# aiven/tiered-storage-for-apache-kafka

Hardware: AMD Instinct MI355X
Metric: GiB/s segment chunk transform (Zstd+AES+CRC), 4MiB chunks (higher is better)
Workload: dtype u8

## Files before the change

### tiered-storage-for-apache-kafka_amd/csrc/zstd_enc_dev.h

```cpp
#define LANES 64
#define UNI(x) ((uint32_t)__builtin_amdgcn_readfirstlane((uint32_t)(x)))
#ifdef HIPEMU
#define ZS_GLOBAL
#else
#define ZS_GLOBAL __attribute__((address_space(1)))
#endif
typedef const ZS_GLOBAL uint8_t* gbytes_t;
typedef ZS_GLOBAL uint32_t* gwords_t;
struct __attribute__((packed)) zs_u64u { uint64_t v; };
struct __attribute__((packed)) zs_u32u { uint32_t v; };
__device__ static inline uint64_t gld64(gbytes_t p) { return reinterpret_cast<const ZS_GLOBAL zs_u64u*>(p)->v; }
__device__ static inline uint32_t gld32(gbytes_t p) { return reinterpret_cast<const ZS_GLOBAL zs_u32u*>(p)->v; }
__device__ static inline uint4 ld128a(const uint8_t* p) { return *reinterpret_cast<const uint4*>(p); }
#ifdef HIPEMU
__device__ static inline void zs_put_seq(zs_seq* p, uint32_t offBase, uint32_t litLength, uint32_t mlBase, uint32_t litPos) { zs_seq q; q.offBase = offBase; q.litLength = litLength; q.mlBase = mlBase; q.litPos = litPos; *p = q; }
#else
typedef uint32_t zs_u32x4 __attribute__((ext_vector_type(4)));
__device__ static inline uint4 ld128a(gbytes_t p) { const zs_u32x4 t = *reinterpret_cast<const ZS_GLOBAL zs_u32x4*>(p); return make_uint4(t.x, t.y, t.z, t.w); }
__device__ static inline void zs_put_seq(ZS_GLOBAL zs_seq* p, uint32_t offBase, uint32_t litLength, uint32_t mlBase, uint32_t litPos) {
    zs_u32x4 t; t.x = offBase; t.y = litLength; t.z = mlBase; t.w = litPos;
    *reinterpret_cast<ZS_GLOBAL zs_u32x4*>(p) = t;
}
#endif
template <class T> __device__ static inline T* uni_ptr(T* p) {
// ... 4 lines not shown
#define ZS_RING 4096u
#define ZS_RWM (ZS_RING / 4 - 1)
#define ZS_FILL 2048u
#define ZS_SAFE 384u
#ifndef ZS_WAVES_PER_SIMD
#define ZS_WAVES_PER_SIMD 6
#endif
#define ZS_SCR 1024u
#define ZS_NOINLINE __attribute__((noinline))

#ifdef TSX_PROF
__shared__ unsigned long long g_prof[24];
__shared__ unsigned long long g_prof_take;
static unsigned long long* g_prof_out = nullptr;
extern "C" void tsx_debug_set_prof(void* dev_ptr) { g_prof_out = (unsigned long long*)dev_ptr; }
#define ZS_PROF_PARAM , unsigned long long* __restrict__ prof_out
#define ZS_PROF_ARG , prof_out
#define ZS_PROF_LAUNCH_ARG , g_prof_out
#else
#define ZS_PROF_PARAM
#define ZS_PROF_ARG
#define ZS_PROF_LAUNCH_ARG
#endif
#if defined(TSX_PROF) && !defined(TSX_PROF2)
#define PT(k) do { const unsigned long long now_ = (unsigned long long)clock64(); if (threadIdx.x == 0) { g_prof[k] += now_ - g_prof[23]; g_prof[23] = now_; } } while (0)
#define PCNT(k, v) do { if (threadIdx.x == 0) g_prof[k] += (v); } while (0)
#define PTW(k) do { asm volatile("s_waitcnt vmcnt(0) lgkmcnt(0)" ::: "memory"); PT(k); } while (0)
#else
#define PT(k) do {} while (0)
#define PCNT(k, v) do {} while (0)
#define PTW(k) do {} while (0)
#endif

__device__ static const uint8_t kLLbits[36] = {0,0,0,0,0,0,0,0,0,0,0,0,0,0,0,0,1,1,1,1,2,2,3,3,4,6,7,8,9,10,11,12,13,14,15,16};
__device__ static const uint8_t kMLbits[53] = {0,0,0,0,0,0,0,0,0,0,0,0,0,0,0,0,0,0,0,0,0,0,0,0,0,0,0,0,0,0,0,0,1,1,1,1,2,2,3,3,4,4,5,7,8,9,10,11,12,13,14,15,16};
__device__ static const short kLLdefaultNorm[36] = {4,3,2,2,2,2,2,2,2,2,2,2,2,1,1,1,2,2,2,2,2,2,2,2,2,3,2,1,1,1,1,1,-1,-1,-1,-1};
__device__ static const short kOFdefaultNorm[29] = {1,1,1,1,1,1,2,2,2,1,1,1,1,1,1,1,1,1,1,1,1,1,1,1,-1,-1,-1,-1,-1};
__device__ static const short kMLdefaultNorm[53] = {1,4,3,2,2,2,2,2,2,1,1,1,1,1,1,1,1,1,1,1,1,1,1,1,1,1,1,1,1,1,1,1,1,1,1,1,1,1,1,1,1,1,1,1,1,1,-1,-1,-1,-1,-1,-1,-1};
__device__ static const uint8_t kLLcode[64] = {0,1,2,3,4,5,6,7,8,9,10,11,12,13,14,15,16,16,17,17,18,18,19,19,20,20,20,20,21,21,21,21,
    22,22,22,22,22,22,22,22,23,23,23,23,23,23,23,23,24,24,24,24,24,24,24,24,24,24,24,24,24,24,24,24};
__device__ static const uint8_t kMLcode[128] = {0,1,2,3,4,5,6,7,8,9,10,11,12,13,14,15,16,17,18,19,20,21,22,23,24,25,26,27,28,29,30,31,
    32,32,33,33,34,34,35,35,36,36,36,36,37,37,37,37,38,38,38,38,38,38,38,38,39,39,39,39,39,39,39,39,
    40,40,40,40,40,40,40,40,40,40,40,40,40,40,40,40,41,41,41,41,41,41,41,41,41,41,41,41,41,41,41,41,
    42,42,42,42,42,42,42,42,42,42,42,42,42,42,42,42,42,42,42,42,42,42,42,42,42,42,42,42,42,42,42,42};
__device__ static const uint32_t kRtb[8] = {0, 473195, 504333, 520860, 550000, 700000, 750000, 830000};

__device__ static inline uint32_t hb32(uint32_t v) { return 31u - (uint32_t)__clz((int)v); }
__device__ static inline uint64_t ld64(const uint8_t* p) { uint64_t v; __builtin_memcpy(&v, p, 8); return v; }
__device__ static inline uint32_t LLcode(uint32_t ll) { return ll > 63 ? hb32(ll) + 19 : kLLcode[ll]; }
__device__ static inline uint32_t MLcode(uint32_t ml) { return ml > 127 ? hb32(ml) + 36 : kMLcode[ml]; }

struct HufTable { uint16_t val[256]; uint8_t nb[256]; uint32_t tableLog, maxSym; };
struct FseTable { uint16_t state[512]; uint32_t dnb[56]; int32_t dfs[56]; uint32_t tableLog; };

enum {
    ZS_SCAL_HUF_HSIZE = 0,
    ZS_SCAL_HUF_USEOLD = 1,
    ZS_SCAL_HUF_FAIL = 2,
    ZS_SCAL_SEQ_QOFF = 3,
    ZS_SCAL_SEQ_COUNTSIZE = 4,
    ZS_SCAL_HUF_BC = 4,
    ZS_SCAL_NEWHUF = 8,
    ZS_SCAL_MULT = 15
};
struct EncLds {
    int hufRepeat[2];
    uint32_t scal[16];
    union alignas(16) {
        struct {
            union { FseTable ll; HufTable huf[2]; };
            FseTable of;
            union {
                FseTable ml;
                uint32_t hist[256];
            };
            uint32_t hist2[256];
            uint8_t tableSymbol[512];
            uint16_t cumul[64];
            short norm[64];
        };
        struct {
            uint32_t ring[ZS_RING / 4 + 4];
            uint8_t scr[2 * ZS_SCR];
        } p;
        struct {
            tsx_gf128 tab[256];
            uint32_t t0[256];
        } g;
        uint32_t crcTab[4 * 256];
    };
};

#ifdef HIPEMU
// ... 24 lines not shown
```

### tiered-storage-for-apache-kafka_amd/csrc/zstd_enc_entropy.h

```cpp
struct BitW { uint8_t* start; uint8_t* p; uint8_t* end; uint64_t acc; uint32_t n; bool overflow; };
__device__ static inline void bw_init(BitW& b, uint8_t* dst, uint8_t* end) { b.start = b.p = dst; b.end = end; b.acc = 0; b.n = 0; b.overflow = false; }
__device__ static inline void bw_add(BitW& b, uint64_t v, uint32_t nb) {
    if (!nb) return;
    b.acc |= (v & ((1ull << nb) - 1)) << b.n;
    b.n += nb;
    while (b.n >= 8) { if (b.p < b.end) *b.p++ = (uint8_t)b.acc; else b.overflow = true; b.acc >>= 8; b.n -= 8; }
}
__device__ static inline uint32_t bw_close(BitW& b) {
    bw_add(b, 1, 1);
    if (b.n) { if (b.p < b.end) *b.p++ = (uint8_t)b.acc; else b.overflow = true; b.n = 0; }
    return (uint32_t)(b.p - b.start);
}

__device__ static uint32_t fse_minTableLog(uint32_t srcSize, uint32_t maxSym) {
    uint32_t a = hb32(srcSize) + 1, b = hb32(maxSym) + 2;
    return a < b ? a : b;
}
__device__ static uint32_t fse_optimalTableLog(uint32_t maxTableLog, uint32_t srcSize, uint32_t maxSym, uint32_t minus) {
    uint32_t maxBitsSrc = hb32(srcSize - 1) - minus, tableLog = maxTableLog, minBits = fse_minTableLog(srcSize, maxSym);
    if (maxBitsSrc < tableLog) tableLog = maxBitsSrc;
    if (minBits > tableLog) tableLog = minBits;
    if (tableLog < 5) tableLog = 5;
    if (tableLog > 12) tableLog = 12;
    return tableLog;
// ... 73 lines not shown
    uint32_t bitStream = 0; int bitCount = 0; uint32_t symbol = 0; const uint32_t alphabetSize = maxSym + 1; int previousIs0 = 0;
    bitStream += (tableLog - 5) << bitCount; bitCount += 4;
    remaining = tableSize + 1; threshold = tableSize; nbBits = (int)tableLog + 1;
    while (symbol < alphabetSize && remaining > 1) {
        if (previousIs0) {
            uint32_t start = symbol;
            while (symbol < alphabetSize && !norm[symbol]) symbol++;
            if (symbol == alphabetSize) break;
            while (symbol >= start + 24) { start += 24; bitStream += 0xFFFFU << bitCount; out[0] = (uint8_t)bitStream; out[1] = (uint8_t)(bitStream >> 8); out += 2; bitStream >>= 16; }
            while (symbol >= start + 3) { start += 3; bitStream += 3U << bitCount; bitCount += 2; }
            bitStream += (symbol - start) << bitCount; bitCount += 2;
            if (bitCount > 16) { out[0] = (uint8_t)bitStream; out[1] = (uint8_t)(bitStream >> 8); out += 2; bitStream >>= 16; bitCount -= 16; }
        }
        {   int c = norm[symbol++];
            const int mx = (2 * threshold - 1) - remaining;
            remaining -= c < 0 ? -c : c;
            c++;
            if (c >= threshold) c += mx;
            bitStream += (uint32_t)c << bitCount;
            bitCount += nbBits;
            bitCount -= (c < mx);
            previousIs0 = (c == 1);
            if (remaining < 1) return 0;
            while (remaining < threshold) { nbBits--; threshold >>= 1; }
        }
        if (bitCount > 16) { out[0] = (uint8_t)bitStream; out[1] = (uint8_t)(bitStream >> 8); out += 2; bitStream >>= 16; bitCount -= 16; }
    }
    if (remaining != 1) return 0;
    out[0] = (uint8_t)bitStream; out[1] = (uint8_t)(bitStream >> 8);
    out += (bitCount + 7) / 8;
    return (uint32_t)(out - out0);
}

__device__ ZS_NOINLINE static void fse_buildCTable(FseTable& ct, const short* norm, uint32_t maxSym, uint32_t tableLog, uint16_t* cumul, uint8_t* tableSymbol) {
    const uint32_t tableSize = 1u << tableLog, tableMask = tableSize - 1, step = (tableSize >> 1) + (tableSize >> 3) + 3;
    uint32_t highThreshold = tableSize - 1, u;
    ct.tableLog = tableLog;
    cumul[0] = 0;
    for (u = 1; u <= maxSym + 1; u++) {
        if (norm[u - 1] == -1) { cumul[u] = (uint16_t)(cumul[u - 1] + 1); tableSymbol[highThreshold--] = (uint8_t)(u - 1); }
        else cumul[u] = (uint16_t)(cumul[u - 1] + (uint32_t)norm[u - 1]);
    }
    cumul[maxSym + 1] = (uint16_t)(tableSize + 1);
    {   uint32_t position = 0;
        for (uint32_t symbol = 0; symbol <= maxSym; symbol++) {
            const int freq = norm[symbol];
            for (int n = 0; n < freq; n++) {
                tableSymbol[position] = (uint8_t)symbol;
                position = (position + step) & tableMask;
                while (position > highThreshold) position = (position + step) & tableMask;
            }
        }
    }
    for (u = 0; u < tableSize; u++) { const uint8_t s = tableSymbol[u]; ct.state[cumul[s]++] = (uint16_t)(tableSize + u); }
    {   uint32_t total = 0;
        for (uint32_t s = 0; s <= maxSym; s++) {
            const int nv = norm[s];
            if (nv == 0) { ct.dnb[s] = ((tableLog + 1) << 16) - (1u << tableLog); ct.dfs[s] = 0; }
            else if (nv == -1 || nv == 1) { ct.dnb[s] = (tableLog << 16) - (1u << tableLog); ct.dfs[s] = (int)(total - 1); total++; }
            else {
                const uint32_t maxBitsOut = tableLog - hb32((uint32_t)nv - 1), minStatePlus = (uint32_t)nv << maxBitsOut;
                ct.dnb[s] = (maxBitsOut << 16) - minStatePlus; ct.dfs[s] = (int)(total - (uint32_t)nv); total += (uint32_t)nv;
            }
        }
    }
}
__device__ static inline uint32_t fse_init2(const FseTable& ct, uint32_t symbol) {
    const uint32_t dnb = ct.dnb[symbol];
    const uint32_t nbBitsOut = (dnb + (1u << 15)) >> 16;
    const uint32_t value = (nbBitsOut << 16) - dnb;
    return ct.state[(value >> nbBitsOut) + ct.dfs[symbol]];
}
__device__ static inline void fse_encode(BitW& b, const FseTable& ct, uint32_t& value, uint32_t symbol) {
    const uint32_t nbBitsOut = (value + ct.dnb[symbol]) >> 16;
    bw_add(b, value, nbBitsOut);
    value = ct.state[(value >> nbBitsOut) + ct.dfs[symbol]];
}

__device__ ZS_NOINLINE static uint32_t huf_writeCTable(uint8_t* dst, const HufTable& ct, uint32_t maxSym, uint32_t huffLog, EncLds& L) {
    uint8_t* const hw = reinterpret_cast<uint8_t*>(L.hist2);
    for (uint32_t n = 0; n < maxSym; n++) { const uint32_t nb = ct.nb[n]; hw[n] = nb ? (uint8_t)(huffLog + 1 - nb) : 0; }
    uint32_t hSize = 0;
    {
        uint8_t* op = dst + 1; const uint32_t wtSize = maxSym;
        uint32_t maxSV = ZS_HUF_TABLELOG_MAX; uint32_t* cnt = L.hist2 + 68;
        if (wtSize > 1) {
// ... 13 lines not shown
                else {
                    BitW b; bw_init(b, op, op + 512);
                    const uint8_t* ip = hw + wtSize; uint32_t s1, s2;
                    if (wtSize & 1) { s1 = fse_init2(L.of, *--ip); s2 = fse_init2(L.of, *--ip); fse_encode(b, L.of, s1, *--ip); }
                    else { s2 = fse_init2(L.of, *--ip); s1 = fse_init2(L.of, *--ip); }
                    while (ip > hw) { fse_encode(b, L.of, s2, *--ip); if (ip > hw) fse_encode(b, L.of, s1, *--ip); }
                    bw_add(b, s2, tableLog); bw_add(b, s1, tableLog);
                    op += bw_close(b);
                    hSize = (uint32_t)(op - (dst + 1));
                }
            }
        }
    }
    if ((hSize > 1) & (hSize < maxSym / 2)) { dst[0] = (uint8_t)hSize; return hSize + 1; }
    if (maxSym > 128) return 0xFFFFFFFFu;
    dst[0] = (uint8_t)(128 + (maxSym - 1));
    hw[maxSym] = 0;
    for (uint32_t n = 0; n < maxSym; n += 2) dst[(n / 2) + 1] = (uint8_t)((hw[n] << 4) + hw[n + 1]);
    return ((maxSym + 1) / 2) + 1;
}

__device__ ZS_NOINLINE static void wave_histogram(uint32_t* hist, const uint8_t* __restrict__ p, uint32_t n, uint32_t lane) {
    for (uint32_t i = lane; i < 256; i += LANES) hist[i] = 0;
    __syncthreads();
    for (uint32_t i = lane; i < n; i += LANES) atomicAdd(&hist[p[i]], 1u);
    __syncthreads();
}

struct WavePack { uint32_t r0, r1, startBit; uint32_t* tmp; uint64_t acc; uint32_t word, nacc; };
__device__ __forceinline__ static void wp_range(WavePack& p, uint32_t n, uint32_t lane) {
    const uint32_t per = (n + LANES - 1) / LANES;
    p.r0 = lane * per < n ? lane * per : n; p.r1 = p.r0 + per < n ? p.r0 + per : n;
}
__device__ __forceinline__ static uint32_t wp_scan(WavePack& p, uint32_t bits, uint32_t lane) {
    if (lane == LANES - 1) bits++;
    p.startBit = wave_excl_scan(bits, lane);
    return __shfl(p.startBit + bits, LANES - 1);
}
__device__ __forceinline__ static void wp_begin(WavePack& p, uint32_t* __restrict__ tmp, uint32_t totalBits, uint32_t lane) {
    const uint32_t words = (totalBits + 31) / 32;
    for (uint32_t w = lane; w < words; w += LANES) tmp[w] = 0;
    stage_sync();
    p.tmp = tmp; p.acc = 0; p.word = p.startBit >> 5; p.nacc = p.startBit & 31;
}
__device__ __forceinline__ static void wp_put(WavePack& p, uint64_t v, uint32_t nb) {
    p.acc |= v << p.nacc;
    p.nacc += nb;
    if (p.nacc >= 32) { atomicOr(&p.tmp[p.word], (uint32_t)p.acc); p.acc >>= 32; p.nacc -= 32; p.word++; }
}
__device__ __forceinline__ static void wp_finish(WavePack& p, uint32_t lane) {
    if (lane == LANES - 1) wp_put(p, 1, 1);
    if (p.nacc) atomicOr(&p.tmp[p.word], (uint32_t)p.acc);
    stage_sync();
}

__device__ ZS_NOINLINE static uint32_t wave_huf_encode(uint32_t* __restrict__ tmp, const uint8_t* __restrict__ src, uint32_t n, const HufTable& ct, uint32_t lane) {
    WavePack p;
    wp_range(p, n, lane);
    uint32_t bits = 0;
    for (uint32_t r = p.r0; r < p.r1; r++) bits += ct.nb[src[n - 1 - r]];
    const uint32_t total = wp_scan(p, bits, lane);
    wp_begin(p, tmp, total, lane);
    for (uint32_t r = p.r0; r < p.r1; r++) {
        const uint8_t s = src[n - 1 - r];
        wp_put(p, ct.val[s], ct.nb[s]);
    }
    wp_finish(p, lane);
    return (total + 7) / 8;
}

__device__ ZS_NOINLINE static uint32_t wave_huf_compress(uint8_t* ostart, uint8_t* op, const uint8_t* __restrict__ lit, uint32_t n, bool single, const HufTable& ct,
                                             uint32_t* tmp, uint32_t lane) {
    if (single) {
        const uint32_t c = wave_huf_encode(tmp, lit, n, ct, lane);
        wave_copy(op, (const uint8_t*)tmp, c, lane);
        op += c;
    } else {
        if (n < 12) return 0;
        const uint32_t seg = (n + 3) / 4;
        uint8_t* const jump = op;
        op += 6;
        for (int i = 0; i < 4; i++) {
            const uint32_t len = i < 3 ? seg : n - 3 * seg;
            const uint32_t c = wave_huf_encode(tmp, lit + (uint32_t)i * seg, len, ct, lane);
            if (c == 0 || c > 65535) return 0;
            if (i < 3 && lane == 0) put_le(jump + 2 * i, c, 2);
// ... 84 lines not shown
                L.scal[ZS_SCAL_HUF_HSIZE] = hSize; L.scal[ZS_SCAL_HUF_USEOLD] = useOld; L.scal[ZS_SCAL_HUF_FAIL] = fail;
            }
            __syncthreads();
            const uint32_t hSize = L.scal[ZS_SCAL_HUF_HSIZE]; const bool useOld = L.scal[ZS_SCAL_HUF_USEOLD], fail = L.scal[ZS_SCAL_HUF_FAIL];
            __syncthreads();
            PT(6);
            if (fail) cLit = 0;
            else if (useOld) { cLit = wave_huf_compress(ostart, ostart, lit, n, single, L.huf[cur], tmp, lane); usedOld = true; }
            else { cLit = wave_huf_compress(ostart, ostart + hSize, lit, n, single, L.huf[nxt], tmp, lane); newTable = true; }
        }
    }
    PT(7);
    const uint32_t minGain = (n >> 6) + 2;
    if (cLit == 0 || cLit >= n - minGain) return write_plain_literals(dst, lit, n, 0, lane);
    if (cLit == 1) return write_plain_literals(dst, lit, n, 1, lane);
    const uint32_t hType = (usedOld && !newTable) ? 3u : 2u;
    if (newTable) L.scal[ZS_SCAL_NEWHUF] = 1;
    if (lane == 0) {
        const uint32_t fmt = lhSize == 3 ? (uint32_t)!single : lhSize - 2, sizeBits = 10 + 4 * (lhSize - 3);
        put_le(dst, hType + (fmt << 2) + ((uint64_t)n << 4) + ((uint64_t)cLit << (4 + sizeBits)), lhSize);
    }
    return lhSize + cLit;
}

__device__ static int select_encoding(uint32_t mostFrequent, uint32_t nbSeq, uint32_t defaultNormLog, bool defaultAllowed, uint32_t mult) {
    if (mostFrequent == nbSeq) return (defaultAllowed && nbSeq <= 2) ? 0 : 1;
    if (defaultAllowed) {
        const uint32_t dynMin = ((1u << defaultNormLog) * mult) >> 3;
        if (nbSeq < dynMin || mostFrequent < (nbSeq >> (defaultNormLog - 1))) return 0;
    }
    return 2;
}

__device__ ZS_NOINLINE static uint32_t build_seq_table(uint8_t* op, FseTable& ct, uint32_t FSELog, uint32_t* cnt, uint32_t maxSymStart, const uint8_t* codes, uint32_t nbSeq,
                                           const short* defaultNorm, uint32_t defaultNormLog, uint32_t defaultMax, bool isOffsets, EncLds& L, uint32_t* type) {
    uint32_t max = maxSymStart;
    while (!cnt[max]) max--;
    uint32_t mostFrequent = 0;
    for (uint32_t s = 0; s <= max; s++) if (cnt[s] > mostFrequent) mostFrequent = cnt[s];
    const bool defaultAllowed = isOffsets ? (max <= ZS_DefaultMaxOff) : true;
    const int t = select_encoding(mostFrequent, nbSeq, defaultNormLog, defaultAllowed, L.scal[ZS_SCAL_MULT]);
    *type = (uint32_t)t;
    if (t == 1) {
        ct.tableLog = 0; ct.state[0] = 0; ct.state[1] = 0; ct.dnb[max] = 0; ct.dfs[max] = 0;
        *op = codes[0];
        return 1;
    }
    if (t == 0) {
        for (uint32_t s = 0; s <= defaultMax; s++) L.norm[s] = defaultNorm[s];
        fse_buildCTable(ct, L.norm, defaultMax, defaultNormLog, L.cumul, L.tableSymbol);
        return 0;
    }
    uint32_t nbSeq_1 = nbSeq;
    const uint32_t tableLog = fse_optimalTableLog(FSELog, nbSeq, max, 2);
    if (cnt[codes[nbSeq - 1]] > 1) { cnt[codes[nbSeq - 1]]--; nbSeq_1--; }
    if (fse_normalizeCount(L.norm, tableLog, cnt, nbSeq_1, max, nbSeq_1 >= 2048) < 0) return 0xFFFFFFFFu;
    const uint32_t sz = fse_writeNCount(op, L.norm, max, tableLog);
    fse_buildCTable(ct, L.norm, max, tableLog, L.cumul, L.tableSymbol);
    return sz;
}

__device__ ZS_NOINLINE static uint32_t compress_sequences(uint8_t* op0, uint8_t* oend, const zs_seq* __restrict__ seqs, uint32_t nbSeq, uint8_t* __restrict__ codes,
                                              EncLds& L, uint32_t* tmp, uint32_t tmpCap, uint32_t lane) {
    uint8_t* op = op0;
    uint8_t* const llC = codes; uint8_t* const ofC = codes + ZS_WS_CODE_STRIDE; uint8_t* const mlC = codes + 2 * ZS_WS_CODE_STRIDE;
    const uint32_t nbSeqBytes = nbSeq < 128 ? 1 : nbSeq < 0x7F00 ? 2 : 3;
    if (lane == 0) put_le(op, nbSeqBytes == 1 ? nbSeq : nbSeqBytes == 2 ? ((nbSeq >> 8) + 0x80) | ((nbSeq & 0xFF) << 8) : 0xFF | ((nbSeq - 0x7F00) << 8), nbSeqBytes);
    op += nbSeqBytes;
    if (nbSeq == 0) return (uint32_t)(op - op0);
    uint32_t* const cLL = L.hist2; uint32_t* const cOF = L.hist2 + 64; uint32_t* const cML = L.hist2 + 128;
    for (uint32_t i = lane; i < 192; i += LANES) L.hist2[i] = 0;
    __syncthreads();
    for (uint32_t u = lane; u < nbSeq; u += LANES) {
        const zs_seq q = seqs[u];
        const uint32_t a = LLcode(q.litLength), b = hb32(q.offBase), c = MLcode(q.mlBase);
        llC[u] = (uint8_t)a; ofC[u] = (uint8_t)b; mlC[u] = (uint8_t)c;
        atomicAdd(&cLL[a], 1u); atomicAdd(&cOF[b], 1u); atomicAdd(&cML[c], 1u);
    }
    stage_sync();
    PT(8);
    if (lane == 0) {
        uint8_t* const seqHead = op; uint8_t* q = op + 1;
        const struct { FseTable* ct; uint32_t fseLog; uint32_t* cnt; uint32_t maxSym; const uint8_t* codes; const short* defNorm; uint32_t defLog, defMax; bool isOffsets; } tabs[3] = {
            {&L.ll, ZS_LLFSELog, cLL, ZS_MaxLL, llC, kLLdefaultNorm, 6, ZS_MaxLL, false},
            {&L.of, ZS_OffFSELog, cOF, ZS_MaxOff, ofC, kOFdefaultNorm, 5, ZS_DefaultMaxOff, true},
            {&L.ml, ZS_MLFSELog, cML, ZS_MaxML, mlC, kMLdefaultNorm, 6, ZS_MaxML, false}};
        uint32_t type[3] = {0, 0, 0}, lastCountSize = 0, fail = 0;
#pragma unroll
        for (int k = 0; k < 3; k++) {
            if (fail) continue;
            const uint32_t sz = build_seq_table(q, *tabs[k].ct, tabs[k].fseLog, tabs[k].cnt, tabs[k].maxSym, tabs[k].codes, nbSeq, tabs[k].defNorm, tabs[k].defLog,
                                                tabs[k].defMax, tabs[k].isOffsets, L, &type[k]);
            if (sz == 0xFFFFFFFFu) { fail = 1; continue; }
            if (type[k] == 2) lastCountSize = sz;
            q += sz;
        }
        L.scal[ZS_SCAL_SEQ_QOFF] = fail ? 0xFFFFFFFFu : (uint32_t)(q - op0);
        L.scal[ZS_SCAL_SEQ_COUNTSIZE] = lastCountSize;
        if (!fail) *seqHead = (uint8_t)((type[0] << 6) + (type[1] << 4) + (type[2] << 2));
        PT(9);
    }
    stage_sync();
    const uint32_t qoff = L.scal[ZS_SCAL_SEQ_QOFF], lastCountSize = L.scal[ZS_SCAL_SEQ_COUNTSIZE];
    __syncthreads();
    if (qoff == 0xFFFFFFFFu) return 0xFFFFFFFFu;
    uint16_t* const stb = (uint16_t*)(codes + 3 * ZS_WS_CODE_STRIDE);
    uint32_t finalState = 0, finalLog = 0;
    if (lane < 3) {
        const FseTable& ct = lane == 0 ? L.ll : lane == 1 ? L.of : L.ml;
        const uint8_t* __restrict__ cd = codes + lane * ZS_WS_CODE_STRIDE;
        uint16_t* __restrict__ o = stb + lane * ZS_WS_CODE_STRIDE;
        uint32_t st = fse_init2(ct, cd[nbSeq - 1]);
        o[nbSeq - 1] = 0;
        if (nbSeq >= 2) {
            int32_t n = (int32_t)nbSeq - 2;
            uint32_t g = (uint32_t)n & ~7u;
            uint64_t cur = *reinterpret_cast<const uint64_t*>(cd + g);
            for (;;) {
                const uint64_t nxt = g >= 8 ? *reinterpret_cast<const uint64_t*>(cd + g - 8) : 0;
                const int top = n & 7;
                uint32_t dn[8]; int32_t df[8];
#pragma unroll
                for (int j = 0; j < 8; j++) { const uint32_t sym = (uint32_t)(cur >> (8 * j)) & 0xFF; dn[j] = ct.dnb[sym < 56 ? sym : 0]; df[j] = ct.dfs[sym < 56 ? sym : 0]; }
                uint32_t ob[4] = {0, 0, 0, 0};
#pragma unroll
                for (int j = 7; j >= 0; j--) {
                    if (j <= top) {
                        const uint32_t nb = (st + dn[j]) >> 16;
                        ob[j >> 1] |= ((st & ((1u << nb) - 1)) | (nb << 12)) << (16 * (j & 1));
                        st = ct.state[(st >> nb) + df[j]];
                    }
                }
                if (top == 7) *reinterpret_cast<uint4*>(o + g) = make_uint4(ob[0], ob[1], ob[2], ob[3]);
                else {
#pragma unroll
                    for (int j = 0; j < 8; j++) if (j <= top) o[g + j] = (uint16_t)(ob[j >> 1] >> (16 * (j & 1)));
                }
                if (g == 0) break;
                g -= 8; n = (int32_t)g + 7; cur = nxt;
            }
        }
        finalState = st & ((1u << ct.tableLog) - 1); finalLog = ct.tableLog;
    }
    stage_sync();
    PT(10);
    const uint32_t fLL = __shfl(finalState, 0), fOF = __shfl(finalState, 1), fML = __shfl(finalState, 2);
    const uint32_t gLL = __shfl(finalLog, 0), gOF = __shfl(finalLog, 1), gML = __shfl(finalLog, 2);
    WavePack p;
    wp_range(p, nbSeq, lane);
    uint32_t bits = 0;
    for (uint32_t r = p.r0; r < p.r1; r++) {
        const uint32_t n = nbSeq - 1 - r;
        bits += (stb[n] >> 12) + (stb[ZS_WS_CODE_STRIDE + n] >> 12) + (stb[2 * ZS_WS_CODE_STRIDE + n] >> 12) + kLLbits[llC[n]] + kMLbits[mlC[n]] + ofC[n];
    }
    if (lane == LANES - 1) bits += gML + gOF + gLL;
    const uint32_t totalBits = wp_scan(p, bits, lane);
    const uint32_t bitstreamSize = (totalBits + 7) / 8;
    uint8_t* const q = op0 + qoff;
    if (q + bitstreamSize > oend || bitstreamSize > tmpCap) return 0xFFFFFFFFu;
    wp_begin(p, tmp, totalBits, lane);
    for (uint32_t r = p.r0; r < p.r1; r++) {
        const uint32_t n = nbSeq - 1 - r;
        const zs_seq sq = seqs[n];
        const uint32_t lc = llC[n], oc = ofC[n], mc = mlC[n];
        const uint32_t sLL = stb[n], sOF = stb[ZS_WS_CODE_STRIDE + n], sML = stb[2 * ZS_WS_CODE_STRIDE + n];
        const uint32_t nOF = sOF >> 12, nML = sML >> 12, nLL = sLL >> 12;
        const uint32_t v1 = (sOF & 0xFFF) | ((sML & 0xFFF) << nOF) | ((sLL & 0xFFF) << (nOF + nML));
        wp_put(p, v1, nOF + nML + nLL);
        const uint32_t bl = kLLbits[lc], bm = kMLbits[mc];
        const uint64_t v2 = (uint64_t)(sq.litLength & ((1u << bl) - 1)) | ((uint64_t)(sq.mlBase & ((1u << bm) - 1)) << bl);
        wp_put(p, v2, bl + bm);
        wp_put(p, sq.offBase & (uint32_t)((1ull << oc) - 1), oc);
    }
    if (lane == LANES - 1) { wp_put(p, fML, gML); wp_put(p, fOF, gOF); wp_put(p, fLL, gLL); }
    wp_finish(p, lane);
    wave_copy(q, (const uint8_t*)tmp, bitstreamSize, lane);
    stage_sync();
    PT(10);
    if (lastCountSize && (lastCountSize + bitstreamSize) < 4) return 0xFFFFFFFFu;
    return qoff + bitstreamSize;
}

__device__ static inline void copy_run(uint8_t* __restrict__ dst, const uint8_t* __restrict__ src, uint32_t n) {
    uint32_t k = 0;
    while (n - k >= 32) {
        const uint64_t a = ld64(src + k), b = ld64(src + k + 8), c = ld64(src + k + 16), d = ld64(src + k + 24);
        __builtin_memcpy(dst + k, &a, 8); __builtin_memcpy(dst + k + 8, &b, 8); __builtin_memcpy(dst + k + 16, &c, 8); __builtin_memcpy(dst + k + 24, &d, 8);
        k += 32;
    }
    const uint32_t r = n - k, nq = r >> 3;
    uint64_t q0 = 0, q1 = 0, q2 = 0; uint32_t w = 0; uint16_t h = 0; uint8_t b1 = 0;
    if (nq > 0) q0 = ld64(src + k);
    if (nq > 1) q1 = ld64(src + k + 8);
    if (nq > 2) q2 = ld64(src + k + 16);
    const uint32_t t = k + 8 * nq;
    if (r & 4) __builtin_memcpy(&w, src + t, 4);
    if (r & 2) __builtin_memcpy(&h, src + t + (r & 4), 2);
    if (r & 1) b1 = src[t + (r & 6)];
    if (nq > 0) __builtin_memcpy(dst + k, &q0, 8);
    if (nq > 1) __builtin_memcpy(dst + k + 8, &q1, 8);
    if (nq > 2) __builtin_memcpy(dst + k + 16, &q2, 8);
    if (r & 4) __builtin_memcpy(dst + t, &w, 4);
    if (r & 2) __builtin_memcpy(dst + t + (r & 4), &h, 2);
    if (r & 1) dst[t + (r & 6)] = b1;
}

__device__ ZS_NOINLINE static void gather_literals(uint8_t* __restrict__ lit, const uint8_t* __restrict__ src, const zs_seq* __restrict__ seqs,
                                                   uint32_t nbSeq, uint32_t tailPos, uint32_t tailLen, uint32_t lane) {
    uint32_t base = 0;
    for (uint32_t g = 0; g < nbSeq; g += LANES) {
// ... 12 lines not shown
```

Measured before the change: 20.17.

## Wave-parallelize FSE table build and stream sequence encoding in 64-seq rounds

Moves the sequence FSE table construction (normalizeCount, CTable build, symbol spread) from a single lane to wave-cooperative code using ballots, scans and shuffles. Sequence encoding now runs in rounds of 64 sequences, staging per-round state transitions in LDS instead of writing a global state buffer. The bitstream is packed incrementally with running bit offsets. This removes serial single-lane work and a global round trip. It adds per-round wave syncs and more complex LDS aliasing.

```diff
diff --git a/tiered-storage-for-apache-kafka_amd/csrc/zstd_enc_dev.h b/tiered-storage-for-apache-kafka_amd/csrc/zstd_enc_dev.h
--- a/tiered-storage-for-apache-kafka_amd/csrc/zstd_enc_dev.h
+++ b/tiered-storage-for-apache-kafka_amd/csrc/zstd_enc_dev.h
@@ -60,8 +60,6 @@
 #define PTW(k) do {} while (0)
 #endif
 
-__device__ static const uint8_t kLLbits[36] = {0,0,0,0,0,0,0,0,0,0,0,0,0,0,0,0,1,1,1,1,2,2,3,3,4,6,7,8,9,10,11,12,13,14,15,16};
-__device__ static const uint8_t kMLbits[53] = {0,0,0,0,0,0,0,0,0,0,0,0,0,0,0,0,0,0,0,0,0,0,0,0,0,0,0,0,0,0,0,0,1,1,1,1,2,2,3,3,4,4,5,7,8,9,10,11,12,13,14,15,16};
 __device__ static const short kLLdefaultNorm[36] = {4,3,2,2,2,2,2,2,2,2,2,2,2,1,1,1,2,2,2,2,2,2,2,2,2,3,2,1,1,1,1,1,-1,-1,-1,-1};
 __device__ static const short kOFdefaultNorm[29] = {1,1,1,1,1,1,2,2,2,1,1,1,1,1,1,1,1,1,1,1,1,1,1,1,-1,-1,-1,-1,-1};
 __device__ static const short kMLdefaultNorm[53] = {1,4,3,2,2,2,2,2,2,1,1,1,1,1,1,1,1,1,1,1,1,1,1,1,1,1,1,1,1,1,1,1,1,1,1,1,1,1,1,1,1,1,1,1,1,1,-1,-1,-1,-1,-1,-1,-1};
@@ -85,8 +83,6 @@
     ZS_SCAL_HUF_HSIZE = 0,
     ZS_SCAL_HUF_USEOLD = 1,
     ZS_SCAL_HUF_FAIL = 2,
-    ZS_SCAL_SEQ_QOFF = 3,
-    ZS_SCAL_SEQ_COUNTSIZE = 4,
     ZS_SCAL_HUF_BC = 4,
     ZS_SCAL_NEWHUF = 8,
     ZS_SCAL_MULT = 15
diff --git a/tiered-storage-for-apache-kafka_amd/csrc/zstd_enc_entropy.h b/tiered-storage-for-apache-kafka_amd/csrc/zstd_enc_entropy.h
--- a/tiered-storage-for-apache-kafka_amd/csrc/zstd_enc_entropy.h
+++ b/tiered-storage-for-apache-kafka_amd/csrc/zstd_enc_entropy.h
@@ -129,6 +129,18 @@
     return (uint32_t)(out - out0);
 }
 
+__device__ static inline void fse_spread_walk(uint8_t* tableSymbol, const short* norm, uint32_t maxSym, uint32_t tableMask, uint32_t step, uint32_t highThreshold) {
+    uint32_t position = 0;
+    for (uint32_t symbol = 0; symbol <= maxSym; symbol++) {
+        const int freq = norm[symbol];
+        for (int n = 0; n < freq; n++) {
+            tableSymbol[position] = (uint8_t)symbol;
+            position = (position + step) & tableMask;
+            while (position > highThreshold) position = (position + step) & tableMask;
+        }
+    }
+}
+
 __device__ ZS_NOINLINE static void fse_buildCTable(FseTable& ct, const short* norm, uint32_t maxSym, uint32_t tableLog, uint16_t* cumul, uint8_t* tableSymbol) {
     const uint32_t tableSize = 1u << tableLog, tableMask = tableSize - 1, step = (tableSize >> 1) + (tableSize >> 3) + 3;
     uint32_t highThreshold = tableSize - 1, u;
@@ -139,16 +151,7 @@
         else cumul[u] = (uint16_t)(cumul[u - 1] + (uint32_t)norm[u - 1]);
     }
     cumul[maxSym + 1] = (uint16_t)(tableSize + 1);
-    {   uint32_t position = 0;
-        for (uint32_t symbol = 0; symbol <= maxSym; symbol++) {
-            const int freq = norm[symbol];
-            for (int n = 0; n < freq; n++) {
-                tableSymbol[position] = (uint8_t)symbol;
-                position = (position + step) & tableMask;
-                while (position > highThreshold) position = (position + step) & tableMask;
-            }
-        }
-    }
+    fse_spread_walk(tableSymbol, norm, maxSym, tableMask, step, highThreshold);
     for (u = 0; u < tableSize; u++) { const uint8_t s = tableSymbol[u]; ct.state[cumul[s]++] = (uint16_t)(tableSize + u); }
     {   uint32_t total = 0;
         for (uint32_t s = 0; s <= maxSym; s++) {
@@ -228,15 +231,15 @@
     const uint32_t per = (n + LANES - 1) / LANES;
     p.r0 = lane * per < n ? lane * per : n; p.r1 = p.r0 + per < n ? p.r0 + per : n;
 }
-__device__ __forceinline__ static uint32_t wp_scan(WavePack& p, uint32_t bits, uint32_t lane) {
-    if (lane == LANES - 1) bits++;
-    p.startBit = wave_excl_scan(bits, lane);
+__device__ __forceinline__ static uint32_t wp_scan(WavePack& p, uint32_t bits, uint32_t lane, uint32_t base = 0, bool last = true) {
+    if (last && lane == LANES - 1) bits++;
+    p.startBit = base + wave_excl_scan(bits, lane);
     return __shfl(p.startBit + bits, LANES - 1);
 }
-__device__ __forceinline__ static void wp_begin(WavePack& p, uint32_t* __restrict__ tmp, uint32_t totalBits, uint32_t lane) {
+__device__ __forceinline__ static void wp_begin(WavePack& p, uint32_t* __restrict__ tmp, uint32_t totalBits, uint32_t lane, uint32_t base = 0) {
     const uint32_t words = (totalBits + 31) / 32;
-    for (uint32_t w = lane; w < words; w += LANES) tmp[w] = 0;
-    stage_sync();
+    for (uint32_t w = (base + 31) / 32 + lane; w < words; w += LANES) tmp[w] = 0;
+    WAVE_MEM_SYNC();
     p.tmp = tmp; p.acc = 0; p.word = p.startBit >> 5; p.nacc = p.startBit & 31;
 }
 __device__ __forceinline__ static void wp_put(WavePack& p, uint64_t v, uint32_t nb) {
@@ -244,10 +247,10 @@
     p.nacc += nb;
     if (p.nacc >= 32) { atomicOr(&p.tmp[p.word], (uint32_t)p.acc); p.acc >>= 32; p.nacc -= 32; p.word++; }
 }
-__device__ __forceinline__ static void wp_finish(WavePack& p, uint32_t lane) {
-    if (lane == LANES - 1) wp_put(p, 1, 1);
+__device__ __forceinline__ static void wp_finish(WavePack& p, uint32_t lane, bool last = true) {
+    if (last && lane == LANES - 1) wp_put(p, 1, 1);
     if (p.nacc) atomicOr(&p.tmp[p.word], (uint32_t)p.acc);
-    stage_sync();
+    if (last) stage_sync();
 }
 
 __device__ ZS_NOINLINE static uint32_t wave_huf_encode(uint32_t* __restrict__ tmp, const uint8_t* __restrict__ src, uint32_t n, const HufTable& ct, uint32_t lane) {
@@ -398,36 +401,212 @@
     return 2;
 }
 
+__device__ ZS_NOINLINE static int wave_fse_normalizeCount(short* norm, uint32_t tableLog, const uint32_t* cnt, uint32_t total, uint32_t maxSym, bool useLowProb, uint32_t lane) {
+    const short lowProbCount = useLowProb ? -1 : 1;
+    const uint64_t scale = 62 - tableLog, step = ((uint64_t)1 << 62) / total, vStep = 1ULL << (scale - 20);
+    const uint32_t lowThreshold = total >> tableLog;
+    if (tableLog < fse_minTableLog(total, maxSym)) return -1;
+    const uint32_t c = lane <= maxSym ? cnt[lane] : 0;
+    if (__any(c == total)) return 0;
+    short n = 0; uint32_t used = 0, proba = 0;
+    if (c != 0 && c <= lowThreshold) { n = lowProbCount; used = 1; }
+    else if (c != 0) {
+        short p = (short)((c * step) >> scale);
+        if (p < 8) { const uint64_t restToBeat = vStep * kRtb[p]; p += (c * step) - ((uint64_t)p << scale) > restToBeat; }
+        n = p; used = proba = (uint32_t)p;
+    }
+    const int still = (1 << tableLog) - (int)wave_sum(used);
+    const uint32_t largestP = wave_max(proba);
+    const uint32_t largest = largestP ? (uint32_t)__ffsll((long long)__ballot(proba == largestP)) - 1 : 0;
+    const int normLargest = __shfl((int)n, (int)largest);
+    const bool m2 = -still >= (normLargest >> 1);
+    if (!m2 && lane == largest) n += (short)still;
+    if (lane <= maxSym) norm[lane] = n;
+    WAVE_MEM_SYNC();
+    if (m2) {
+        int r = 0;
+        if (lane == 0) r = fse_normalizeM2(norm, tableLog, cnt, total, maxSym, lowProbCount);
+        WAVE_MEM_SYNC();
+        if (__shfl(r, 0) < 0) return -1;
+    }
+    return (int)tableLog;
+}
+
+__device__ __forceinline__ static uint32_t lanes_below(uint64_t ballot) { return __builtin_amdgcn_mbcnt_hi((uint32_t)(ballot >> 32), __builtin_amdgcn_mbcnt_lo((uint32_t)ballot, 0)); }
+
+__device__ ZS_NOINLINE static void wave_fse_buildCTable(FseTable& ct, const short* norm, uint32_t maxSym, uint32_t tableLog, uint8_t* tableSymbol, uint32_t lane) {
+    const uint32_t tableSize = 1u << tableLog, tableMask = tableSize - 1, step = (tableSize >> 1) + (tableSize >> 3) + 3;
+    const int nv = lane <= maxSym ? norm[lane] : 0;
+    const uint32_t occ = nv == -1 ? 1u : (uint32_t)nv;
+    uint32_t cum = wave_excl_scan(occ, lane);
+    if (lane == 0) ct.tableLog = tableLog;
+    if (lane <= maxSym) {
+        if (occ == 0) { ct.dnb[lane] = ((tableLog + 1) << 16) - tableSize; ct.dfs[lane] = 0; }
+        else {
+            const uint32_t maxBitsOut = tableLog - (occ > 1 ? hb32(occ - 1) : 0), minStatePlus = occ << maxBitsOut;
+            ct.dnb[lane] = (maxBitsOut << 16) - minStatePlus; ct.dfs[lane] = (int)(cum - occ);
+        }
+    }
+    const uint64_t low = __ballot(nv == -1);
+    if (low) {
+        if (nv == -1) tableSymbol[tableMask - lanes_below(low)] = (uint8_t)lane;
+        if (lane == 0) fse_spread_walk(tableSymbol, norm, maxSym, tableMask, step, tableMask - (uint32_t)__popcll(low));
+    } else {
+#pragma unroll 1
+        for (uint32_t s = 0; s <= maxSym; s++) {
+            const uint32_t f = __shfl(occ, (int)s), first = __shfl(cum, (int)s);
+#pragma unroll 1
+            for (uint32_t k = lane; k < f; k += LANES) tableSymbol[((first + k) * step) & tableMask] = (uint8_t)s;
+        }
+    }
+    WAVE_MEM_SYNC();
+#pragma unroll 1
+    for (uint32_t u0 = 0; u0 < tableSize; u0 += LANES) {
+        const uint32_t u = u0 + lane;
+        const bool valid = u < tableSize;
+        const uint32_t sym = valid ? tableSymbol[u] : 0;
+        uint64_t todo = __ballot(valid);
+        while (todo) {
+            const uint32_t s0 = __shfl(sym, __ffsll((long long)todo) - 1);
+            const bool mine = valid && sym == s0;
+            const uint64_t m = __ballot(mine);
+            const uint32_t first = __shfl(cum, (int)s0);
+            if (mine) ct.state[first + lanes_below(m)] = (uint16_t)(tableSize + u);
+            if (lane == s0) cum += (uint32_t)__popcll(m);
+            todo &= ~m;
+        }
+    }
+}
+
 __device__ ZS_NOINLINE static uint32_t build_seq_table(uint8_t* op, FseTable& ct, uint32_t FSELog, uint32_t* cnt, uint32_t maxSymStart, const uint8_t* codes, uint32_t nbSeq,
-                                           const short* defaultNorm, uint32_t defaultNormLog, uint32_t defaultMax, bool isOffsets, EncLds& L, uint32_t* type) {
-    uint32_t max = maxSymStart;
-    while (!cnt[max]) max--;
-    uint32_t mostFrequent = 0;
-    for (uint32_t s = 0; s <= max; s++) if (cnt[s] > mostFrequent) mostFrequent = cnt[s];
+                                           const short* defaultNorm, uint32_t defaultNormLog, uint32_t defaultMax, bool isOffsets, EncLds& L, uint32_t* type, uint32_t lane) {
+    const uint32_t c = lane <= maxSymStart ? cnt[lane] : 0;
+    const uint32_t max = UNI(wave_max(c ? lane : 0)), mostFrequent = UNI(wave_max(c));
     const bool defaultAllowed = isOffsets ? (max <= ZS_DefaultMaxOff) : true;
     const int t = select_encoding(mostFrequent, nbSeq, defaultNormLog, defaultAllowed, L.scal[ZS_SCAL_MULT]);
     *type = (uint32_t)t;
     if (t == 1) {
-        ct.tableLog = 0; ct.state[0] = 0; ct.state[1] = 0; ct.dnb[max] = 0; ct.dfs[max] = 0;
-        *op = codes[0];
+        if (lane == 0) { ct.tableLog = 0; ct.state[0] = 0; ct.state[1] = 0; ct.dnb[max] = 0; ct.dfs[max] = 0; *op = codes[0]; }
         return 1;
     }
     if (t == 0) {
-        for (uint32_t s = 0; s <= defaultMax; s++) L.norm[s] = defaultNorm[s];
-        fse_buildCTable(ct, L.norm, defaultMax, defaultNormLog, L.cumul, L.tableSymbol);
+        if (lane <= defaultMax) L.norm[lane] = defaultNorm[lane];
+        WAVE_MEM_SYNC();
+        wave_fse_buildCTable(ct, L.norm, defaultMax, defaultNormLog, L.tableSymbol, lane);
         return 0;
     }
     uint32_t nbSeq_1 = nbSeq;
     const uint32_t tableLog = fse_optimalTableLog(FSELog, nbSeq, max, 2);
-    if (cnt[codes[nbSeq - 1]] > 1) { cnt[codes[nbSeq - 1]]--; nbSeq_1--; }
-    if (fse_normalizeCount(L.norm, tableLog, cnt, nbSeq_1, max, nbSeq_1 >= 2048) < 0) return 0xFFFFFFFFu;
-    const uint32_t sz = fse_writeNCount(op, L.norm, max, tableLog);
-    fse_buildCTable(ct, L.norm, max, tableLog, L.cumul, L.tableSymbol);
+    const uint32_t lastCode = codes[nbSeq - 1];
+    if (UNI(cnt[lastCode]) > 1) {
+        nbSeq_1--;
+        WAVE_MEM_SYNC();
+        if (lane == 0) cnt[lastCode]--;
+        WAVE_MEM_SYNC();
+    }
+    if (wave_fse_normalizeCount(L.norm, tableLog, cnt, nbSeq_1, max, nbSeq_1 >= 2048, lane) < 0) return 0xFFFFFFFFu;
+    uint32_t sz = 0;
+    if (lane == 0) sz = fse_writeNCount(op, L.norm, max, tableLog);
+    sz = __shfl(sz, 0);
+    wave_fse_buildCTable(ct, L.norm, max, tableLog, L.tableSymbol, lane);
     return sz;
 }
 
-__device__ ZS_NOINLINE static uint32_t compress_sequences(uint8_t* op0, uint8_t* oend, const zs_seq* __restrict__ seqs, uint32_t nbSeq, uint8_t* __restrict__ codes,
-                                              EncLds& L, uint32_t* tmp, uint32_t tmpCap, uint32_t lane) {
+__device__ __forceinline__ static uint32_t ll_extra_bits(uint32_t c) { return c < 16 ? 0 : c >= 25 ? c - 19 : (uint32_t)(0x433221111ull >> (4 * (c - 16))) & 15; }
+__device__ __forceinline__ static uint32_t ml_extra_bits(uint32_t c) { return c < 32 ? 0 : c >= 43 ? c - 36 : (uint32_t)(0x54433221111ull >> (4 * (c - 32))) & 15; }
+
+#define ZS_SEQ_STG_STRIDE 65u
+__device__ __forceinline__ static uint32_t fse_chain_round(const FseTable& ct, uint2* __restrict__ e, uint32_t cnt, uint32_t st, bool first) {
+    uint32_t g = 0;
+    if (first) {
+        const uint2 d = e[0];
+        const uint32_t nb = (d.x + (1u << 15)) >> 16;
+        st = ct.state[(((nb << 16) - d.x) >> nb) + (int32_t)d.y];
+        e[0].x = 0;
+        g = 1;
+    }
+    for (; g < cnt; g += 8) {
+        uint2 d[8]; uint32_t o[8];
+#pragma unroll
+        for (int j = 0; j < 8; j++) d[j] = g + j < cnt ? e[g + j] : make_uint2(0, 0);
+#pragma unroll
+        for (int j = 0; j < 8; j++) {
+            if (g + j < cnt) {
+                const uint32_t nb = (st + d[j].x) >> 16;
+                o[j] = (st & ((1u << nb) - 1)) | (nb << 12);
+                st = ct.state[(st >> nb) + (int32_t)d[j].y];
+            }
+        }
+#pragma unroll
+        for (int j = 0; j < 8; j++) if (g + j < cnt) e[g + j].x = o[j];
+    }
+    return st;
+}
+
+__device__ __forceinline__ static uint32_t encode_sequences(uint8_t* q_, uint32_t cap_, const zs_seq* __restrict__ seqs_, uint32_t nbSeq_, const uint8_t* __restrict__ codes_, EncLds& L,
+                                                        uint32_t* tmp_, uint32_t lane) {
+    uint8_t* const q = uni_ptr(q_); const zs_seq* __restrict__ const seqs = uni_ptr(seqs_); const uint8_t* __restrict__ const codes = uni_ptr(codes_); uint32_t* const tmp = uni_ptr(tmp_);
+    const uint32_t cap = UNI(cap_), nbSeq = UNI(nbSeq_);
+    static_assert(offsetof(EncLds, tableSymbol) == offsetof(EncLds, hist2) + sizeof(((EncLds*)0)->hist2) && offsetof(EncLds, cumul) == offsetof(EncLds, tableSymbol) + sizeof(((EncLds*)0)->tableSymbol) &&
+                  3 * ZS_SEQ_STG_STRIDE * sizeof(uint2) <= sizeof(((EncLds*)0)->hist2) + sizeof(((EncLds*)0)->tableSymbol) + sizeof(((EncLds*)0)->cumul) && (offsetof(EncLds, hist2) & 7) == 0,
+                  "the round's staging fits what the table constructions have left behind: hist2, tableSymbol, cumul");
+    const uint8_t* const llC = codes; const uint8_t* const ofC = codes + ZS_WS_CODE_STRIDE; const uint8_t* const mlC = codes + 2 * ZS_WS_CODE_STRIDE;
+    uint2* const stg = reinterpret_cast<uint2*>(L.hist2);
+    const FseTable& ct = lane == 1 ? L.of : lane == 2 ? L.ml : L.ll;
+    uint2* const chain = stg + (lane < 3 ? lane : 0) * ZS_SEQ_STG_STRIDE;
+    uint32_t st = 0, base = 0;
+    zs_seq sq = {0, 0, 0, 0}; uint32_t lc = 0, oc = 0, mc = 0;
+    if (lane < nbSeq) { const uint32_t n = nbSeq - 1 - lane; sq = seqs[n]; lc = llC[n]; oc = ofC[n]; mc = mlC[n]; }
+    for (uint32_t r0 = 0; r0 < nbSeq; r0 += LANES) {
+        const uint32_t cnt = nbSeq - r0 < LANES ? nbSeq - r0 : LANES;
+        const bool last = r0 + LANES >= nbSeq, valid = lane < cnt;
+        if (valid) {
+            stg[lane] = make_uint2(L.ll.dnb[lc], (uint32_t)L.ll.dfs[lc]);
+            stg[ZS_SEQ_STG_STRIDE + lane] = make_uint2(L.of.dnb[oc], (uint32_t)L.of.dfs[oc]);
+            stg[2 * ZS_SEQ_STG_STRIDE + lane] = make_uint2(L.ml.dnb[mc], (uint32_t)L.ml.dfs[mc]);
+        }
+        const uint32_t bl = ll_extra_bits(lc), bm = ml_extra_bits(mc), n2 = bl + bm, n3 = oc;
+        const uint32_t x2 = (sq.litLength & ((1u << bl) - 1)) | ((sq.mlBase & ((1u << bm) - 1)) << bl);
+        const uint32_t x3 = sq.offBase & (uint32_t)((1ull << oc) - 1);
+        if (r0 + LANES + lane < nbSeq) { const uint32_t n = nbSeq - 1 - (r0 + LANES + lane); sq = seqs[n]; lc = llC[n]; oc = ofC[n]; mc = mlC[n]; }
+        WAVE_MEM_SYNC();
+        if (lane < 3) st = fse_chain_round(ct, chain, cnt, st, r0 == 0);
+        WAVE_MEM_SYNC();
+        uint32_t x1 = 0, n1 = 0;
+        if (valid) {
+            const uint32_t sLL = stg[lane].x, sOF = stg[ZS_SEQ_STG_STRIDE + lane].x, sML = stg[2 * ZS_SEQ_STG_STRIDE + lane].x;
+            const uint32_t nOF = sOF >> 12, nML = sML >> 12, nLL = sLL >> 12;
+            x1 = (sOF & 0xFFF) | ((sML & 0xFFF) << nOF) | ((sLL & 0xFFF) << (nOF + nML));
+            n1 = nOF + nML + nLL;
+        }
+        uint32_t bits = valid ? n1 + n2 + n3 : 0;
+        uint32_t fLL = 0, fOF = 0, fML = 0, gLL = 0, gOF = 0, gML = 0;
+        if (last) {
+            const uint32_t fin = st & ((1u << ct.tableLog) - 1);
+            fLL = __shfl(fin, 0); fOF = __shfl(fin, 1); fML = __shfl(fin, 2);
+            gLL = L.ll.tableLog; gOF = L.of.tableLog; gML = L.ml.tableLog;
+            if (lane == LANES - 1) bits += gML + gOF + gLL;
+        }
+        WavePack p;
+        const uint32_t total = wp_scan(p, bits, lane, base, last);
+        if ((total + 7) / 8 > cap) return 0xFFFFFFFFu;
+        wp_begin(p, tmp, total, lane, base);
+        if (valid) { wp_put(p, x1, n1); wp_put(p, x2, n2); wp_put(p, x3, n3); }
+        if (last && lane == LANES - 1) { wp_put(p, fML, gML); wp_put(p, fOF, gOF); wp_put(p, fLL, gLL); }
+        wp_finish(p, lane, last);
+        base = total;
+    }
+    const uint32_t bitstreamSize = (base + 7) / 8;
+    wave_copy(q, (const uint8_t*)tmp, bitstreamSize, lane);
+    stage_sync();
+    return bitstreamSize;
+}
+
+__device__ ZS_NOINLINE static uint32_t compress_sequences(uint8_t* op0_, uint8_t* oend_, const zs_seq* __restrict__ seqs_, uint32_t nbSeq_, uint8_t* __restrict__ codes_,
+                                              EncLds& L, uint32_t* tmp_, uint32_t tmpCap_, uint32_t lane) {
+    uint8_t* const op0 = uni_ptr(op0_); uint8_t* const oend = uni_ptr(oend_); const zs_seq* __restrict__ const seqs = uni_ptr(seqs_); uint8_t* __restrict__ const codes = uni_ptr(codes_);
+    uint32_t* const tmp = uni_ptr(tmp_);
+    const uint32_t nbSeq = UNI(nbSeq_), tmpCap = UNI(tmpCap_);
     uint8_t* op = op0;
     uint8_t* const llC = codes; uint8_t* const ofC = codes + ZS_WS_CODE_STRIDE; uint8_t* const mlC = codes + 2 * ZS_WS_CODE_STRIDE;
     const uint32_t nbSeqBytes = nbSeq < 128 ? 1 : nbSeq < 0x7F00 ? 2 : 3;
@@ -445,103 +624,33 @@
     }
     stage_sync();
     PT(8);
-    if (lane == 0) {
-        uint8_t* const seqHead = op; uint8_t* q = op + 1;
+    uint32_t qoff, lastCountSize = 0;
+    {   uint8_t* const seqHead = op; uint8_t* q = op + 1;
         const struct { FseTable* ct; uint32_t fseLog; uint32_t* cnt; uint32_t maxSym; const uint8_t* codes; const short* defNorm; uint32_t defLog, defMax; bool isOffsets; } tabs[3] = {
             {&L.ll, ZS_LLFSELog, cLL, ZS_MaxLL, llC, kLLdefaultNorm, 6, ZS_MaxLL, false},
             {&L.of, ZS_OffFSELog, cOF, ZS_MaxOff, ofC, kOFdefaultNorm, 5, ZS_DefaultMaxOff, true},
             {&L.ml, ZS_MLFSELog, cML, ZS_MaxML, mlC, kMLdefaultNorm, 6, ZS_MaxML, false}};
-        uint32_t type[3] = {0, 0, 0}, lastCountSize = 0, fail = 0;
+        uint32_t type[3] = {0, 0, 0}, fail = 0;
 #pragma unroll
         for (int k = 0; k < 3; k++) {
             if (fail) continue;
-            const uint32_t sz = build_seq_table(q, *tabs[k].ct, tabs[k].fseLog, tabs[k].cnt, tabs[k].maxSym, tabs[k].codes, nbSeq, tabs[k].defNorm, tabs[k].defLog,
-                                                tabs[k].defMax, tabs[k].isOffsets, L, &type[k]);
+            const uint32_t sz = UNI(build_seq_table(q, *tabs[k].ct, tabs[k].fseLog, tabs[k].cnt, tabs[k].maxSym, tabs[k].codes, nbSeq, tabs[k].defNorm, tabs[k].defLog,
+                                                    tabs[k].defMax, tabs[k].isOffsets, L, &type[k], lane));
+            type[k] = UNI(type[k]);
             if (sz == 0xFFFFFFFFu) { fail = 1; continue; }
             if (type[k] == 2) lastCountSize = sz;
             q += sz;
         }
-        L.scal[ZS_SCAL_SEQ_QOFF] = fail ? 0xFFFFFFFFu : (uint32_t)(q - op0);
-        L.scal[ZS_SCAL_SEQ_COUNTSIZE] = lastCountSize;
-        if (!fail) *seqHead = (uint8_t)((type[0] << 6) + (type[1] << 4) + (type[2] << 2));
+        qoff = fail ? 0xFFFFFFFFu : (uint32_t)(q - op0);
+        if (!fail && lane == 0) *seqHead = (uint8_t)((type[0] << 6) + (type[1] << 4) + (type[2] << 2));
         PT(9);
     }
     stage_sync();
-    const uint32_t qoff = L.scal[ZS_SCAL_SEQ_QOFF], lastCountSize = L.scal[ZS_SCAL_SEQ_COUNTSIZE];
-    __syncthreads();
     if (qoff == 0xFFFFFFFFu) return 0xFFFFFFFFu;
-    uint16_t* const stb = (uint16_t*)(codes + 3 * ZS_WS_CODE_STRIDE);
-    uint32_t finalState = 0, finalLog = 0;
-    if (lane < 3) {
-        const FseTable& ct = lane == 0 ? L.ll : lane == 1 ? L.of : L.ml;
-        const uint8_t* __restrict__ cd = codes + lane * ZS_WS_CODE_STRIDE;
-        uint16_t* __restrict__ o = stb + lane * ZS_WS_CODE_STRIDE;
-        uint32_t st = fse_init2(ct, cd[nbSeq - 1]);
-        o[nbSeq - 1] = 0;
-        if (nbSeq >= 2) {
-            int32_t n = (int32_t)nbSeq - 2;
-            uint32_t g = (uint32_t)n & ~7u;
-            uint64_t cur = *reinterpret_cast<const uint64_t*>(cd + g);
-            for (;;) {
-                const uint64_t nxt = g >= 8 ? *reinterpret_cast<const uint64_t*>(cd + g - 8) : 0;
-                const int top = n & 7;
-                uint32_t dn[8]; int32_t df[8];
-#pragma unroll
-                for (int j = 0; j < 8; j++) { const uint32_t sym = (uint32_t)(cur >> (8 * j)) & 0xFF; dn[j] = ct.dnb[sym < 56 ? sym : 0]; df[j] = ct.dfs[sym < 56 ? sym : 0]; }
-                uint32_t ob[4] = {0, 0, 0, 0};
-#pragma unroll
-                for (int j = 7; j >= 0; j--) {
-                    if (j <= top) {
-                        const uint32_t nb = (st + dn[j]) >> 16;
-                        ob[j >> 1] |= ((st & ((1u << nb) - 1)) | (nb << 12)) << (16 * (j & 1));
-                        st = ct.state[(st >> nb) + df[j]];
-                    }
-                }
-                if (top == 7) *reinterpret_cast<uint4*>(o + g) = make_uint4(ob[0], ob[1], ob[2], ob[3]);
-                else {
-#pragma unroll
-                    for (int j = 0; j < 8; j++) if (j <= top) o[g + j] = (uint16_t)(ob[j >> 1] >> (16 * (j & 1)));
-                }
-                if (g == 0) break;
-                g -= 8; n = (int32_t)g + 7; cur = nxt;
-            }
-        }
-        finalState = st & ((1u << ct.tableLog) - 1); finalLog = ct.tableLog;
-    }
-    stage_sync();
-    PT(10);
-    const uint32_t fLL = __shfl(finalState, 0), fOF = __shfl(finalState, 1), fML = __shfl(finalState, 2);
-    const uint32_t gLL = __shfl(finalLog, 0), gOF = __shfl(finalLog, 1), gML = __shfl(finalLog, 2);
-    WavePack p;
-    wp_range(p, nbSeq, lane);
-    uint32_t bits = 0;
-    for (uint32_t r = p.r0; r < p.r1; r++) {
-        const uint32_t n = nbSeq - 1 - r;
-        bits += (stb[n] >> 12) + (stb[ZS_WS_CODE_STRIDE + n] >> 12) + (stb[2 * ZS_WS_CODE_STRIDE + n] >> 12) + kLLbits[llC[n]] + kMLbits[mlC[n]] + ofC[n];
-    }
-    if (lane == LANES - 1) bits += gML + gOF + gLL;
-    const uint32_t totalBits = wp_scan(p, bits, lane);
-    const uint32_t bitstreamSize = (totalBits + 7) / 8;
     uint8_t* const q = op0 + qoff;
-    if (q + bitstreamSize > oend || bitstreamSize > tmpCap) return 0xFFFFFFFFu;
-    wp_begin(p, tmp, totalBits, lane);
-    for (uint32_t r = p.r0; r < p.r1; r++) {
-        const uint32_t n = nbSeq - 1 - r;
-        const zs_seq sq = seqs[n];
-        const uint32_t lc = llC[n], oc = ofC[n], mc = mlC[n];
-        const uint32_t sLL = stb[n], sOF = stb[ZS_WS_CODE_STRIDE + n], sML = stb[2 * ZS_WS_CODE_STRIDE + n];
-        const uint32_t nOF = sOF >> 12, nML = sML >> 12, nLL = sLL >> 12;
-        const uint32_t v1 = (sOF & 0xFFF) | ((sML & 0xFFF) << nOF) | ((sLL & 0xFFF) << (nOF + nML));
-        wp_put(p, v1, nOF + nML + nLL);
-        const uint32_t bl = kLLbits[lc], bm = kMLbits[mc];
-        const uint64_t v2 = (uint64_t)(sq.litLength & ((1u << bl) - 1)) | ((uint64_t)(sq.mlBase & ((1u << bm) - 1)) << bl);
-        wp_put(p, v2, bl + bm);
-        wp_put(p, sq.offBase & (uint32_t)((1ull << oc) - 1), oc);
-    }
-    if (lane == LANES - 1) { wp_put(p, fML, gML); wp_put(p, fOF, gOF); wp_put(p, fLL, gLL); }
-    wp_finish(p, lane);
-    wave_copy(q, (const uint8_t*)tmp, bitstreamSize, lane);
-    stage_sync();
+    const uint32_t room = q < oend ? (uint32_t)(oend - q) : 0;
+    const uint32_t bitstreamSize = UNI(encode_sequences(q, room < tmpCap ? room : tmpCap, seqs, nbSeq, codes, L, tmp, lane));
+    if (bitstreamSize == 0xFFFFFFFFu) return 0xFFFFFFFFu;
     PT(10);
     if (lastCountSize && (lastCountSize + bitstreamSize) < 4) return 0xFFFFFFFFu;
     return qoff + bitstreamSize;
```

Result: slower. 17.50 (-13.2%).
